# Gaius-Augustus/Augustus

Measured on AMD Instinct MI355X. Metric: Mbp DNA decoded/sec (whole node), ab-initio human model, higher is better.
Workload: dtype f64; 1 GPU; synthetic uniform-random DNA, 100 contigs x 1000000 bp per GPU, --species=human ab initio (47 states, sample=0); pieces_in_flight_per_gpu=100, batches_in_flight_per_gpu=1

## Files before the change

augustus_amd/csrc/device/decoder.hip:

```cpp
#include <hip/hip_runtime.h>
#include <sys/mman.h>
#include <algorithm>
#include <map>
#include <array>
#include <cmath>
#include <unordered_map>
#include <cstdio>
#include <cstdlib>
#include <cstring>
#include <future>
#include <memory>
#include <mutex>
#include <set>
#include <string>
#include <system_error>
#include <thread>
#include <atomic>
#include <chrono>
#include <vector>
#include "kernels.h"
#include "dense.h"
#include "layout.h"
#include "launch.h"
#include "assmemo.h"
// ... 156 lines not shown
    if (t < NF) {
        uint64_t x = L.w[t][0];
        for (int i = 1; i < SCAN_W; i++) x = t < nSum ? x + L.w[t][i] : (x > L.w[t][i] ? x : L.w[t][i]);
        tot[t] = x;
    }
}
template <int NF> __device__ inline void blockScan(uint64_t (&v)[NF], int nSum, ScanLds<NF> &L, const uint64_t *pre) {
    const int t = threadIdx.x, lane = t & 63, wave = t >> 6;
#pragma unroll
    for (int f = 0; f < NF; f++) {
        const uint64_t x = f < nSum ? waveScanIncl<true>(v[f]) : waveScanIncl<false>(v[f]);
        v[f] = x;
        if (lane == 63) L.w[f][wave] = x;
    }
    __syncthreads();
    if (t < NF) {
        uint64_t acc = pre[t];
        for (int i = 0; i < SCAN_W; i++) {
            const uint64_t x = L.w[t][i];
            L.w[t][i] = acc;
            acc = t < nSum ? acc + x : (acc > x ? acc : x);
        }
    }
    __syncthreads();
#pragma unroll
    for (int f = 0; f < NF; f++) {
        const uint64_t a = L.w[f][wave];
        v[f] = f < nSum ? v[f] + a : (v[f] > a ? v[f] : a);
    }
}
constexpr int NSF = NCNT + 6;
__global__ void __launch_bounds__(SCAN_T) kSiteScanTotals(const DevTables *__restrict__ T, BatchView B, uint64_t *tot ) {
    __shared__ ScanLds<NSF> L;
    __shared__ SlotCodes C;
    C.load(B);
    const int64_t g = (int64_t)blockIdx.x * SCAN_T + threadIdx.x;
    uint64_t v[NSF];
    k1SiteTermsCalc(*T, B, g, v, v + NCNT, C.c, C.lo, C.lo + 256 + 2 * SLOT_HALO);
    blockTotals<NSF>(v, NCNT, L, tot + (int64_t)blockIdx.x * NSF);
}
__global__ void __launch_bounds__(SCAN_T) kSiteScanApply(const DevTables *__restrict__ T, BatchView B, const uint64_t *tot) {
    __shared__ ScanLds<NSF> L;
    __shared__ SlotCodes C;
    C.load(B);
    const int64_t g = (int64_t)blockIdx.x * SCAN_T + threadIdx.x;
    uint64_t v[NSF];
    k1SiteTermsCalc(*T, B, g, v, v + NCNT, C.c, C.lo, C.lo + 256 + 2 * SLOT_HALO);
    blockScan<NSF>(v, NCNT, L, tot + (int64_t)blockIdx.x * NSF);
#pragma unroll
    for (int f = 0; f < NCNT; f++) B.cnt[fidx(g, f, NCNT)] = (uint32_t)v[f];
#pragma unroll
    for (int f = 0; f < 6; f++) B.nsm[fidx(g, f, 6)] = (uint32_t)v[NCNT + f];
}
__global__ void __launch_bounds__(SCAN_T) kFxScanTotals(const DevTables *__restrict__ T, BatchView B, uint64_t *tot ) {
    __shared__ ScanLds<NFX> L;
    __shared__ SlotCodes C;
    C.load(B);
    const int64_t g = (int64_t)blockIdx.x * SCAN_T + threadIdx.x;
    uint64_t v[NFX];
    if (!k1FxTermsCalc(*T, B, g, blockIdx.y, v, C.c, C.lo, C.lo + 256 + 2 * SLOT_HALO)) return;
    blockTotals<NFX>(v, NFX, L, tot + ((int64_t)blockIdx.y * (B.N / SCAN_T) + blockIdx.x) * NFX);
}
__global__ void __launch_bounds__(SCAN_T) kFxScanApply(const DevTables *__restrict__ T, BatchView B, const uint64_t *tot) {
    __shared__ ScanLds<NFX> L;
    __shared__ SlotCodes C;
    C.load(B);
    const int64_t g = (int64_t)blockIdx.x * SCAN_T + threadIdx.x;
    uint64_t v[NFX];
    if (!k1FxTermsCalc(*T, B, g, blockIdx.y, v, C.c, C.lo, C.lo + 256 + 2 * SLOT_HALO)) return;
    blockScan<NFX>(v, NFX, L, tot + ((int64_t)blockIdx.y * (B.N / SCAN_T) + blockIdx.x) * NFX);
    uint64_t *fx = B.fx + (int64_t)blockIdx.y * B.N * NFX;
#pragma unroll
    for (int f = 0; f < NFX; f++) fx[fidx(g, f, NFX)] = v[f];
}
__global__ void __launch_bounds__(64) kChunkOffsets(uint64_t *tot, BatchView B, int nf, int nSum) {
    const int p = blockIdx.x, f = blockIdx.z, lane = threadIdx.x;
    tot += (int64_t)blockIdx.y * (B.N / SCAN_T) * nf;
    const bool sum = f < nSum;
    uint64_t acc = 0;
    const int64_t c1 = B.off[p + 1] / SCAN_T;
    for (int64_t c0 = B.off[p] / SCAN_T; c0 < c1; c0 += 64) {
        const int64_t ch = c0 + lane;
        const uint64_t v = ch < c1 ? tot[ch * nf + f] : 0;
        uint64_t x = v;
        for (int o = 1; o < 64; o <<= 1) {
            const uint64_t y = (uint64_t)__shfl_up((unsigned long long)x, o, 64);
            if (lane >= o) x = sum ? x + y : (x > y ? x : y);
        }
        const uint64_t prev = (uint64_t)__shfl_up((unsigned long long)x, 1, 64);
        const uint64_t ex = lane == 0 ? acc : (sum ? acc + prev : (acc > prev ? acc : prev));
        if (ch < c1) tot[ch * nf + f] = ex;
        const uint64_t last = (uint64_t)__shfl((unsigned long long)x, 63, 64);
        acc = sum ? acc + last : (acc > last ? acc : last);
    }
}

constexpr int NUF = NUFX + NUCNT;
__global__ void __launch_bounds__(SCAN_T) kUtrScanTotals(const DevTables *__restrict__ T, BatchView B, uint64_t *tot ) {
    __shared__ ScanLds<NUF> L;
    __shared__ SlotCodes C;
    C.load(B);
    const int64_t g = (int64_t)blockIdx.x * SCAN_T + threadIdx.x;
    uint64_t v[NUF];
    k1UtrTermsCalc(*T, B, g, v, C.c, C.lo, C.lo + 256 + 2 * SLOT_HALO);
    blockTotals<NUF>(v, NUF, L, tot + (int64_t)blockIdx.x * NUF);
}
__global__ void __launch_bounds__(SCAN_T) kUtrScanApply(const DevTables *__restrict__ T, BatchView B, const uint64_t *tot) {
    __shared__ ScanLds<NUF> L;
    __shared__ SlotCodes C;
    C.load(B);
    const int64_t g = (int64_t)blockIdx.x * SCAN_T + threadIdx.x;
    uint64_t v[NUF];
    k1UtrTermsCalc(*T, B, g, v, C.c, C.lo, C.lo + 256 + 2 * SLOT_HALO);
    blockScan<NUF>(v, NUF, L, tot + (int64_t)blockIdx.x * NUF);
#pragma unroll
    for (int f = 0; f < NUFX; f++) B.ufx[fidx(g, f, NUFX)] = v[f];
#pragma unroll
    for (int f = 0; f < NUCNT; f++) B.ucnt[fidx(g, f, NUCNT)] = (uint32_t)v[NUFX + f];
}
__global__ void kUtrListCount(BatchView B) {
    int p = blockIdx.x * blockDim.x + threadIdx.x;
    if (p < B.nPieces) k1UtrListCount(B, p);
// ... 50 lines not shown
    const int t = threadIdx.x;
    if (t == 0) running = 0;
    __syncthreads();
    for (int base = w.b0; base <= w.b1; base += 256) {
        const int q = base + t;
        const uint32_t cnt = q <= w.b1 ? V.blkCnt[(w.gb0 + q) * 2 + 1] : 0;
        sc[t] = cnt;
        __syncthreads();
        for (int off = 1; off < 256; off <<= 1) {
            const uint32_t v = t >= off ? sc[t - off] : 0;
            __syncthreads();
            sc[t] += v;
            __syncthreads();
        }
        const uint64_t dst = (uint64_t)w.poolOff + running + (sc[t] - cnt);
        if (cnt) {
            const Item *src = V.items + V.blkOff[(w.gb0 + q) * 2 + 1];
            for (uint32_t i = 0; i < cnt; i++) outItems[dst + i] = src[i];
        }
        __syncthreads();
        if (t == 255) running += sc[255];
        __syncthreads();
    }
    const int64_t nFx = (int64_t)w.nPl * 2 * w.nSlots;
    for (int64_t i = t; i < nFx; i += 256) {
        const int pl = (int)(i / (2 * w.nSlots)), rev = (int)((i / w.nSlots) % 2), g = w.g0 + (int)(i % w.nSlots);
        outFx[w.fxOff + i] = V.fx[(int64_t)pl * V.N * NFX + fidx(w.o + g, rev ? FX_INR : FX_INF, NFX)];
    }
    if (mat && outF)
        for (int64_t i = t; i < (int64_t)w.nRows * S; i += 256) outF[w.fOff + i] = mat[(w.o + 1 + w.r0) * S + i];
}
__global__ void __launch_bounds__(256) kPatchItems(BatchView B, const uint64_t *idx, const double *te, int n) {
    const int i = blockIdx.x * blockDim.x + threadIdx.x;
    if (i < n) B.items[idx[i]].te = te[i];
}

namespace augx { namespace dev {
#define AUGX_BY_BLK(f, ...) do { if (blk == 8) f##8(__VA_ARGS__); else if (blk == 4) f##4(__VA_ARGS__); else f##2(__VA_ARGS__); } while (0)
void launchTrellis(int blk, int mode, bool ties, unsigned grid, hipStream_t st, const DevTables *T, const BatchView *B) { AUGX_BY_BLK(launchTrellis_, mode, ties, grid, st, T, B); }
void launchCand(int blk, bool multi, bool dense, unsigned grid, hipStream_t st, const DevTables *T, const BatchView &W) { AUGX_BY_BLK(launchCand_, multi, dense, grid, st, T, W); }
void launchForward(int blk, unsigned grid, hipStream_t st, const DevTables *T, const BatchView *B) { AUGX_BY_BLK(launchForward_, grid, st, T, B); }
void launchDense(int blk, int mode, bool ties, unsigned grid, hipStream_t st, const DevTables *T, const BatchView *B) { AUGX_BY_BLK(launchDense_, mode, ties, grid, st, T, B); }
void launchUtrDesc(int blk, unsigned grid, hipStream_t st, const DevTables *T, const BatchView &W) { AUGX_BY_BLK(launchUtrDesc_, grid, st, T, W); }
#undef AUGX_BY_BLK
}}

struct augx_decoder {
    const augx_model *model = nullptr;
    int device = 0;
    hipStream_t stream = nullptr;
    DevTables hostT;
    DevTables *dT = nullptr;
    std::vector<void *> tableBufs;
    bool debugCells = false;
    int blk = 8;
    int nCU = 256;
    int share = 1;
    std::multimap<size_t, void *> pool;
    std::unordered_map<void *, size_t> live;
    std::atomic<size_t> pooledBytes{0};
    std::mutex poolMu;
    std::vector<hipStream_t> copyStreams;
    bool dense = false;
    bool countNearTies = false;
    int64_t nearTies = 0, nearTiePieces = 0;
    double mallocSeconds = 0, mallocBytes = 0;
    bool exactMulti = true;
};

namespace {
int snippetCacheReplay(augx_decoder *d, augx_batch *b, int64_t &nPatched, bool fromLists, const double *mat);
int utrCachesReplay(augx_decoder *d, augx_batch *b, const double *mat, bool &rebuilt);
std::mutex g_regMu;
std::vector<augx_decoder *> g_decoders;
constexpr size_t POOL_CAP_BYTES = (size_t)250 << 30;
size_t sizeClass(size_t bytes) {
    if (bytes < ((size_t)1 << 20)) return (bytes + 4095) & ~(size_t)4095;
    size_t p2 = (size_t)1 << 20;
    while (p2 < bytes) p2 <<= 1;
    const size_t step = p2 >> 4;
    return (bytes + step - 1) / step * step;
}
void poolReleaseLocked(augx_decoder *d) {
    for (auto &kv : d->pool) (void)hipFree(kv.second);
    d->pool.clear();
    d->pooledBytes = 0;
}
void poolRelease(augx_decoder *d) {
    std::lock_guard<std::mutex> lk(d->poolMu);
    poolReleaseLocked(d);
}
hipError_t devMalloc(augx_decoder *d, void **out, size_t bytes) {
    if (bytes == 0) bytes = 1;
    bytes = sizeClass(bytes);
    {
        std::lock_guard<std::mutex> lk(d->poolMu);
        auto it = d->pool.lower_bound(bytes);
        if (it != d->pool.end() && it->first <= bytes + bytes / 4 + 4096) {
            *out = it->second;
            d->live[*out] = it->first;
            d->pooledBytes -= it->first;
            d->pool.erase(it);
            return hipSuccess;
        }
    }
    const auto tm0 = std::chrono::steady_clock::now();
// ... 134 lines not shown

}

extern "C" {

int augx_device_count(void) {
    int ndev = 0;
    if (hipGetDeviceCount(&ndev) != hipSuccess) { (void)hipGetLastError(); return 0; }
    return ndev;
}

int augx_decoder_create(const augx_model *m, int device, augx_decoder **out) {
    if (!m || !out) { setLastError("augx_decoder_create: NULL argument"); return AUGX_E_ARG; }
    *out = nullptr;
    int ndev = 0;
    hipError_t e = hipGetDeviceCount(&ndev);
    if (e != hipSuccess || ndev <= 0) {
        setLastError("augx_decoder_create: no HIP device available (this library has no CPU decode path)");
        return AUGX_E_NODEVICE;
    }
    if (device < 0 || device >= ndev) { setLastError("augx_decoder_create: bad device index"); return AUGX_E_ARG; }
    const augx_tables &t = m->m.t;
    int blk = 8;
    try {
        blk = chooseBlockSize(t);
    } catch (std::exception &ex) {
        setLastError(ex.what());
        return AUGX_E_UNSUPPORTED;
    }
    HIP_TRY(hipSetDevice(device));
    augx_decoder *d = new augx_decoder();
    d->model = m;
    d->device = device;
    d->blk = blk;
    d->dense = modelIsDense(t);
    d->countNearTies = getenv("AUGX_NEAR_TIES") && atoi(getenv("AUGX_NEAR_TIES")) != 0;
    const char *dbg = getenv("AUGX_DEBUG_CELLS");
    d->debugCells = dbg && atoi(dbg) != 0;
    if (const char *ex = getenv("AUGX_EXACT_MULTICLASS")) d->exactMulti = atoi(ex) != 0;
    { int cu = 0; if (hipDeviceGetAttribute(&cu, hipDeviceAttributeMultiprocessorCount, device) == hipSuccess && cu > 0) d->nCU = cu; else (void)hipGetLastError(); }
    const int rc = [&]() -> int {
        HIP_TRY(hipStreamCreate(&d->stream));
        try { fillDevTablesScalars(t, d->hostT); } catch (std::exception &ex) { setLastError(ex.what()); return AUGX_E_UNSUPPORTED; }
        for (auto &sp : tableSpans(t, d->hostT)) {
            void *p = nullptr;
            size_t bytes = (size_t)(sp.count > 0 ? sp.count : 1) * sizeof(double);
            HIP_TRY(hipMalloc(&p, bytes));
            d->tableBufs.push_back(p);
            if (sp.count > 0) HIP_TRY(hipMemcpy(p, sp.src, (size_t)sp.count * sizeof(double), hipMemcpyHostToDevice));
            *sp.dst = (TabPtr)p;
        }
        HIP_TRY(hipMalloc((void **)&d->dT, sizeof(DevTables)));
        HIP_TRY(hipMemcpy(d->dT, &d->hostT, sizeof(DevTables), hipMemcpyHostToDevice));
        return AUGX_OK;
    }();
    if (rc) { augx_decoder_destroy(d); return rc; }
    { std::lock_guard<std::mutex> rk(g_regMu); g_decoders.push_back(d); }
    *out = d;
    return AUGX_OK;
}

int augx_decoder_set_share(augx_decoder *d, int n) {
    if (!d || n < 1) { setLastError("augx_decoder_set_share: bad argument"); return AUGX_E_ARG; }
    d->share = n;
    return AUGX_OK;
}

int augx_decoder_count_near_ties(augx_decoder *d, int on) { if (!d) return AUGX_E_ARG; d->countNearTies = on != 0; return AUGX_OK; }
int64_t augx_decoder_near_ties(const augx_decoder *d, int64_t *pieces) { if (pieces) *pieces = d ? d->nearTiePieces : 0; return d ? d->nearTies : 0; }
int augx_decoder_exact(const augx_decoder *d) { return d && d->exactMulti ? 1 : 0; }
int augx_decoder_set_exact(augx_decoder *d, int on) {
    if (!d) return AUGX_E_ARG;
    d->exactMulti = on != 0;
    return AUGX_OK;
}

int64_t augx_decoder_batch_capacity(augx_decoder *d) {
    if (!d) return 0;
    size_t freeB = 0, totalB = 0;
    if (hipSetDevice(d->device) != hipSuccess || hipMemGetInfo(&freeB, &totalB) != hipSuccess) return 16L * 1000 * 1000;
    freeB += d->pooledBytes;
    {
        size_t nOn = 0;
        std::lock_guard<std::mutex> rk(g_regMu);
        for (augx_decoder *o : g_decoders) nOn += o->device == d->device;
        if (nOn > 1) freeB = std::min(freeB, (size_t)((double)totalB * 0.9 / (double)nOn));
    }
    int64_t cap = (int64_t)(freeB / (d->dense ? 1500 + 18 * (size_t)d->model->m.t.S : d->model->m.t.n_classes > 1 ? 2000 : 1500));
    if (cap > 128L * 1000 * 1000) cap = 128L * 1000 * 1000;
    if (cap < 1000 * 1000) cap = 1000 * 1000;
    return cap;
}

int64_t augx_decoder_sampled_capacity(augx_decoder *d) {
    const int64_t cap = augx_decoder_batch_capacity(d);
    if (!d || d->dense) return cap;
    const int64_t base = d->model->m.t.n_classes > 1 ? 2000 : 1500;
    return cap * base / (base + 8 * (int64_t)d->model->m.t.S);
}

void augx_release_host_pools();
void augx_decoder_destroy(augx_decoder *d) {
    if (!d) return;
    bool last;
    { std::lock_guard<std::mutex> rk(g_regMu); g_decoders.erase(std::remove(g_decoders.begin(), g_decoders.end(), d), g_decoders.end()); last = g_decoders.empty(); }
    if (last) augx_release_host_pools();
// ... 218 lines not shown
            HIP_TRY(hipMemcpy(planeCls.data(), V.planeCls, sizeof(int32_t) * n * MAXPL, hipMemcpyDeviceToHost));
            std::vector<uint8_t> wc, plane;
            for (int p = 0; p < n; p++) {
                if (cls[p] >= 0) continue;
                const int len = b->L.len[p];
                wc.resize((size_t)len);
                HIP_TRY(hipMemcpy(wc.data(), V.gcRaw + b->L.off[p] + 1, (size_t)len, hipMemcpyDeviceToHost));
                const int np = stairsPlanes(wc.data(), len, d->model->m.t.gc_win, plane, &planeCls[(size_t)p * MAXPL]);
                if (np < 0) continue;
                cls[p] = planeCls[(size_t)p * MAXPL];
                nPlanes[p] = np;
                if (np > nPl) nPl = np;
                if (np > 1) HIP_TRY(hipMemcpy(V.gcPlane + b->L.off[p] + 1, plane.data(), (size_t)len, hipMemcpyHostToDevice));
            }
            HIP_TRY(hipMemcpy(V.cls, cls.data(), sizeof(int32_t) * n, hipMemcpyHostToDevice));
            HIP_TRY(hipMemcpy(V.nPlanes, nPlanes.data(), sizeof(int32_t) * n, hipMemcpyHostToDevice));
            HIP_TRY(hipMemcpy(V.planeCls, planeCls.data(), sizeof(int32_t) * n * MAXPL, hipMemcpyHostToDevice));
        }
        bool changed = W.nPl != nPl;
        if (d->dense && !b->listsReady) {
            utrScan();
            hipLaunchKernelGGL(kUtrListCount, dim3((n + 63) / 64), dim3(64), 0, st, V);
            HIP_TRY(hipGetLastError());
            HIP_TRY(hipStreamSynchronize(st));
        }
        if (!b->listsReady) {
            std::vector<int32_t> lc(n);
            std::vector<int64_t> offs;
            HIP_TRY(hipMemcpy(lc.data(), V.listCnt, sizeof(int32_t) * n, hipMemcpyDeviceToHost));
            W.listCap = listOffsets(lc.data(), n, offs);
            b->hListOffs = offs;
            HIP_TRY(hipMemcpy(b->dListOffs, offs.data(), sizeof(int64_t) * (n + 1), hipMemcpyHostToDevice));
            b->listsReady = true;
            changed = true;
        }
        bool grown = false;
        if (timingFirst) tf[2] = nowS();
        if ((rc = ensureArrays(b, nPl, W.listCap, &grown))) return rc;
        if (timingFirst) tf[3] = nowS();
        if (changed || grown) {
            W.nPl = nPl;
            HIP_TRY(hipMemcpy(b->dV, &W, sizeof(BatchView), hipMemcpyHostToDevice));
        }
    }
    }
    if (V.nPl > b->chunkTotPlanes) {
        DevBuf nt;
        if ((rc = nt.alloc(d, sizeof(uint64_t) * (size_t)V.nPl * (V.N / SCAN_T) * NFX, "augx_batch_decode: out of device memory for the scan totals"))) return rc;
        b->V.chunkTot = nt.as<uint64_t>();
        b->bufs.push_back(std::move(nt));
        b->chunkTotPlanes = V.nPl;
    }
    if (d->dense && !b->utrScanned) utrScan();
    hipLaunchKernelGGL(kFxScanTotals, dim3(nScan, V.nPl), dim3(SCAN_T), 0, st, d->dT, V, V.chunkTot);
    hipLaunchKernelGGL(kChunkOffsets, dim3(n, V.nPl, NFX), dim3(64), 0, st, V.chunkTot, V, NFX, NFX);
    hipLaunchKernelGGL(kFxScanApply, dim3(nScan, V.nPl), dim3(SCAN_T), 0, st, d->dT, V, V.chunkTot);
    hipLaunchKernelGGL(kSignals, dim3(gridN), dim3(256), 0, st, d->dT, V);
    hipLaunchKernelGGL(kSiteSignals, dim3((unsigned)((V.listCap + 255) / 256), 4), dim3(256), 0, st, d->dT, V);
    hipLaunchKernelGGL(kSiteConsts, dim3(gridN, V.nPl), dim3(256), 0, st, d->dT, V);
    if (d->dense) hipLaunchKernelGGL(kUtrSignals, dim3(gridN), dim3(256), 0, st, d->dT, V);
    HIP_TRY(hipGetLastError());
    {
        BatchView &W = b->V;
        const unsigned nWg = (unsigned)(W.N / (WAVE * NWAVES));
        if (b->itemBuf && b->nItems > 0 && (uint64_t)W.itemCap > b->nItems + b->nItems / 16 + 65536) {
            HIP_TRY(hipStreamSynchronize(st));
            b->itemBuf.reset();
            b->itemsVerified = false;
        }
        if (!b->itemBuf) {
            W.itemCap = b->nItems > 0 ? (int64_t)(b->nItems + b->nItems / 16 + 65536) : W.N * 18 + 65536;
            if ((rc = b->itemBuf.alloc(d, (size_t)W.itemCap * sizeof(Item), "augx_batch_decode: out of device memory for the candidate buffer; decode fewer bases per batch"))) return rc;
            W.items = b->itemBuf.as<Item>();
            HIP_TRY(hipMemcpyAsync(b->dV, &W, sizeof(BatchView), hipMemcpyHostToDevice, st));
        }
        const bool utrDesc = d->dense && d->hostT.utr;
        if (utrDesc && !b->udBuf) {
            W.udCap = b->nDescs > 0 ? (int64_t)(b->nDescs + 64) : W.N / 2 + 65536;
            if (const char *e = getenv("AUGX_UD_CAP")) { if (b->nDescs == 0) W.udCap = atol(e) > 0 ? atol(e) : 1; }
            if ((rc = b->udBuf.alloc(d, (size_t)W.udCap * sizeof(UDesc), "augx_batch_decode: out of device memory for the UTR descriptors; decode fewer bases per batch"))) return rc;
            W.ud = b->udBuf.as<UDesc>();
            HIP_TRY(hipMemcpyAsync(b->dV, &W, sizeof(BatchView), hipMemcpyHostToDevice, st));
        }
        const bool steady = b->decoded && b->itemBuf && b->nItems > 0 && (uint64_t)W.itemCap >= b->nItems && b->itemsVerified;
        for (int attempt = 0;; attempt++) {
            HIP_TRY(hipMemsetAsync(W.candAlloc, 0, sizeof(CandAlloc), st));
            const bool multi = W.nPl > 1;
            if (utrDesc) {
                const unsigned nGrp = (unsigned)(W.N / (NT / 16));
                launchUtrDesc(d->blk, nGrp, st, d->dT, W);
            }
            launchCand(d->blk, multi, d->dense, nWg, st, d->dT, W);
            HIP_TRY(hipGetLastError());
            if (steady) break;
            CandAlloc tot;
            HIP_TRY(hipMemcpyAsync(&tot, W.candAlloc, sizeof tot, hipMemcpyDeviceToHost, st));
            HIP_TRY(hipStreamSynchronize(st));
            b->nPairs = tot.pairs; b->nItems = tot.items; b->nDescs = tot.descs;
            const bool itemsFit = (int64_t)tot.items <= W.itemCap, descsFit = !utrDesc || (int64_t)tot.descs <= W.udCap;
            if (itemsFit && descsFit) { b->itemsVerified = true; break; }
            if (attempt > 0) { setLastError("augx_batch_decode: candidate buffers overflowed twice"); return AUGX_E_HIP; }
            if (!itemsFit) {
                W.itemCap = (int64_t)tot.items + 64;
                if ((rc = b->itemBuf.alloc(d, (size_t)W.itemCap * sizeof(Item), "augx_batch_decode: out of device memory for the candidate buffer (" + std::to_string(tot.items) + " candidates); decode fewer bases per batch"))) return rc;
                W.items = b->itemBuf.as<Item>();
            }
            if (!descsFit) {
                W.udCap = (int64_t)tot.descs + 64;
                if ((rc = b->udBuf.alloc(d, (size_t)W.udCap * sizeof(UDesc), "augx_batch_decode: out of device memory for the UTR descriptors; decode fewer bases per batch"))) return rc;
// ... 1017 lines not shown
```

augustus_amd/csrc/device/kernels.h:

```cpp
#pragma once
#include <type_traits>
#include "dp.h"

namespace augx {
namespace dev {

#ifdef AUGX_EMU
#define FOR_LANES(l) for (int l = 0; l < WAVE; ++l)
#define LV(T, name) T name[WAVE]
#define LV2(T, name, K) T name[K][WAVE]
#define LI l
#define LX(name) name[l]
#define WAVE_SYNC() ((void)0)
#define GLOBAL_SYNC() ((void)0)
#define AUGX_KFN inline
#define FOR_THREADS(t) for (int t = 0; t < NT; ++t)
#define FOR_WAVES(w) for (int w = 0; w < NWAVES; ++w)
#define FOR_WLANES(t, w) for (int t = (w) * WAVE; t < (w) * WAVE + WAVE; ++t)
#define TV(T, name) T name[NT]
#define TV2(T, name, K) T name[K][NT]
#define TI t
#define TX(name) name[t]
#define BLOCK_SYNC() ((void)0)
#define BLOCK_GLOBAL_SYNC() ((void)0)
// ... 185 lines not shown
}
AUGX_HD int k1WindowClass(const DevTables &T, const BatchView &B, int64_t g) {
    int p = B.chunkPiece[g / CHUNK];
    int64_t o = B.off[p];
    int s = (int)(g - o - 1), n = B.len[p];
    int win = T.gc_win;
    if (win > n || win < 1) win = n;
    if (s < 0 || s > n - win) return -1;
    if (T.C == 1) { B.gcRaw[g] = 0; return 0; }
    double cnt[4];
    for (int i = 0; i < 4; i++) cnt[i] = (double)(B.cnt[fidx(o + s + win, i, NCNT)] - B.cnt[fidx(o + s, i, NCNT)]);
    if (cnt[0] + cnt[1] + cnt[2] + cnt[3] == 0.0)
        for (int i = 0; i < 4; i++) cnt[i] = (double)(B.cnt[fidx(o + win, i, NCNT)] - B.cnt[fidx(o, i, NCNT)]);
    const int c = nearestClass(T, cnt);
    B.gcRaw[g] = (uint8_t)c;
    return c;
}

AUGX_HD bool k1FxTermsCalc(const DevTables &T, const BatchView &B, int64_t g, int pl, uint64_t out[NFX],
                           const uint8_t *lcode = nullptr, int lLo = 0, int lHi = 0) {
    int p = B.chunkPiece[g / CHUNK];
    if (pl > 0 && pl >= B.nPlanes[p]) return false;
    int64_t o = B.off[p];
    int q = (int)(g - o - 1);
    for (int i = 0; i < NFX; i++) out[i] = 0;
    Piece P;
    P.t = &T; P.n = B.len[p]; P.c = B.cls[p] < 0 ? -1 : B.planeCls[p * MAXPL + pl]; P.o = o; P.code = B.code + o + 1; P.fx = nullptr; P.nsm = nullptr; P.sig = nullptr;
    P.lcode = lcode; P.lLo = lLo; P.lHi = lHi;
    if (q >= 0 && q < B.len[p] && P.c >= 0) {
    const int k = T.k, NP = T.NP, c = P.c;
    int pn = q >= k ? P.pat(q - k, k + 1) : -1;
    int rn = P.rcpat(q, k + 1);
    const double *tabs[3] = {T.ex_emi + (int64_t)c * 3 * NP, T.ex_init + (int64_t)c * 3 * NP, T.ex_et + (int64_t)c * 3 * NP};
    for (int a = 0; a < 3; a++)
        for (int tb = 0; tb < 3; tb++) {
            out[(0 * 3 + a) * 3 + tb] = toFx(pn >= 0 ? tabs[tb][mod3(q + a) * NP + pn] : T.ln_n_coding);
            out[(1 * 3 + a) * 3 + tb] = toFx(rn >= 0 ? tabs[tb][mod3(a - q) * NP + rn] : T.ln_n_coding);
        }
    const double *inE = T.in_emi + (int64_t)c * T.NPin;
    const double softB = (T.soft && B.raw[g] >= 'a' && B.raw[g] <= 'z') ? T.lnSoft : 0.0;
    const int ki = T.kIn;
    const int pni = ki == k ? pn : (q >= ki ? P.pat(q - ki, ki + 1) : -1);
    out[FX_INF] = toFx((pni >= 0 ? inE[pni] : T.ln_quarter) + softB);
    int rn2 = (q + ki < P.n) ? (ki == k ? rn : P.rcpat(q, ki + 1)) : -1;
    out[FX_INR] = toFx((rn2 >= 0 ? inE[rn2] : T.ln_quarter) + softB);
    }
    return true;
}
AUGX_HD void k1FxTerms(const DevTables &T, const BatchView &B, int64_t g, int pl) {
    uint64_t out[NFX];
    if (!k1FxTermsCalc(T, B, g, pl, out)) return;
    uint64_t *fx = B.fx + (int64_t)pl * B.N * NFX;
    for (int i = 0; i < NFX; i++) fx[fidx(g, i, NFX)] = out[i];
}

constexpr int NSITE = 4;
AUGX_HD void k1Signals(const DevTables &T, const BatchView &B, int64_t g, const uint8_t *lcode = nullptr, int lLo = 0, int lHi = 0) {
    int p = B.chunkPiece[g / CHUNK];
    int64_t o = B.off[p];
    int q = (int)(g - o - 1);
    double e[NSIG];
    for (int i = 0; i < NSIG; i++) e[i] = AUGX_NINF;
    int32_t stv[NSITE];
    for (int i = 0; i < NSITE; i++) stv[i] = -1;
    uint64_t gate = 0;
    int64_t atgIdx = -1;
    const bool inPiece = !(q < 0 || q >= B.len[p] || B.cls[p] < 0);
    int64_t lo = 0;
    if (inPiece) {
    Piece P = makePieceAt(T, B, p, B.gcPlane[g]);
    P.lcode = lcode; P.lLo = lLo; P.lHi = lHi;
    const double softB = (T.soft && B.raw[g] >= 'a' && B.raw[g] <= 'z') ? T.lnSoft : 0.0;
    e[SIG_EIG] = q >= 1 ? eIg(P, q) + softB : AUGX_NINF;
    e[SIG_EIN] = eIn(P, q) + softB;
    if (T.utr && T.uk != T.k) e[SIG_EUIN] = eUin(P, q) + softB;
    e[SIG_TISR] = tisRev(P, q);
    e[SIG_STOPF] = exEndPart(P, AUGX_K_TERMINAL, 0, q, AUGX_NINF);
    uint64_t cn[NCNT], cp[NCNT];
    for (int i = CNT_ATG; i < NCNT; i++) { cn[i] = B.cnt[fidx(g, i, NCNT)]; cp[i] = B.cnt[fidx(g - 1, i, NCNT)]; }
    lo = listOff(B, p);
    for (int i = 0; i < NSITE; i++)
        stv[i] = cn[CNT_LA + i] != cp[CNT_LA + i] ? (int32_t)cn[CNT_LA + i] - 1 : -1;
    if (cn[CNT_ATG] != cp[CNT_ATG]) atgIdx = (int64_t)cn[CNT_ATG] - 1;
    if (q - T.dStateLen >= 0) e[SIG_EQD] = P.seg(FX_INF, q - T.dStateLen + 1, q);
    if (q >= 1) {
        const bool stopOpen = e[SIG_STOPF] > AUGX_NINF && q - 3 >= 0;
        const bool tisOpen = e[SIG_TISR] > AUGX_NINF && q - T.W - 3 >= 0;
        bool fwdOpen[3];
        for (int w2 = 0; w2 < 3; w2++) fwdOpen[w2] = exEndPart(P, AUGX_K_INTERNAL, w2, q, AUGX_NINF) > AUGX_NINF;
        const bool revOpen = exEndPart(P, AUGX_K_RINTERNAL, 0, q, AUGX_NINF) > AUGX_NINF;
        const bool lessOpen = lessDGate(P, true, q), rlessOpen = lessDGate(P, false, q);
        for (int s = 0; s < T.S; s++) {
            if (!T.reachable[s]) continue;
            const int kind = T.kind[s], w2 = T.win[s];
            bool open = false;
            switch (kind) {
            case AUGX_K_SINGLE: case AUGX_K_TERMINAL: open = stopOpen; break;
            case AUGX_K_RSINGLE: case AUGX_K_RINITIAL: open = tisOpen; break;
            case AUGX_K_INITIAL: case AUGX_K_INTERNAL: open = w2 == 0 ? fwdOpen[0] : w2 == 1 ? fwdOpen[1] : fwdOpen[2]; break;
            case AUGX_K_RINTERNAL: case AUGX_K_RTERMINAL: open = revOpen; break;
            case AUGX_K_LESSD: open = lessOpen; break;
            case AUGX_K_RLESSD: open = rlessOpen; break;
            default: break;
            }
            if (open) gate |= 1ull << T.vbit[s];
        }
// ... 2565 lines not shown
        }
    }
}

AUGX_KFN void segFinalizePiece(const BatchView &B, int p) {
    const int s0 = B.pieceSeg0[p], K = B.pieceSeg0[p + 1] - s0, n = B.len[p];
    if (K <= 1) {
        B.brkPos[s0] = n - 1; B.brkOff[s0] = 0.0;
        if (B.status[p] == 0 && !(fabs(B.lnv[p]) < AUGX_EXACT_LIMIT)) B.status[p] = AUGX_E_RANGE;
        return;
    }
    double off = 0.0;
    int covered = -1, r = 0;
    bool abortAny = false;
    const int lastTile = (n + WAVE - 1) / WAVE - 1;
    for (int k = 0; k < K; k++)
        if (B.segStatus[s0 + k]) abortAny = true;
    for (int k = 1; k < K; k++) {
        const int st = B.segStop[s0 + k];
        int endTile = st >= -1 ? st : B.segStop2[s0 + k];
        const double D = st >= -1 ? B.segD[s0 + k] : B.segD2[s0 + k];
        if (st < -1 && endTile < 0) { abortAny = true; endTile = lastTile; }
#ifdef AUGX_EMU
        if (endTile < covered - 1) g_emuTrellis[ET_FIN_OVERRUN]++;
        else { g_emuTrellis[ET_FIN_COVERED] += st < -1 && endTile > covered; g_emuTrellis[endTile >= lastTile ? ET_FIN_TO_END : ET_FIN_SEAM]++; }
#endif
        if (endTile < covered - 1) continue;
        if (st < -1 && endTile > covered) covered = endTile;
        if (endTile >= lastTile) break;
        B.brkPos[s0 + r] = (endTile + 1) * WAVE - 1; B.brkOff[s0 + r] = off; r++;
        off = off + D;
    }
    for (; r < K; r++) { B.brkPos[s0 + r] = n - 1; B.brkOff[s0 + r] = off; }
    if (B.status[p] == 0) B.lnv[p] = B.lnv[p] + off;
    if (abortAny) B.status[p] = AUGX_E_HIP;
    if (B.status[p] == 0 && !(fabs(B.lnv[p]) < AUGX_EXACT_LIMIT)) B.status[p] = AUGX_E_RANGE;
}

#ifdef AUGX_EMU
inline int waveCount(const int *flag) { int c = 0; for (int l = 0; l < WAVE; l++) c += flag[l] != 0; return c; }
inline int waveFirstTrue(const int *flag) {
    for (int l = 0; l < WAVE; l++)
        if (flag[l]) return l;
    return WAVE;
}
#else
__device__ inline int waveCount(const int *flag) { return __popcll(__ballot(flag[0] != 0)); }
__device__ inline int waveFirstTrue(const int *flag) {
    unsigned long long m = __ballot(flag[0] != 0);
    return m ? (int)__ffsll((long long)m) - 1 : WAVE;
}
#endif

AUGX_KFN void backtracePiece(const DevTables &T, const BatchView &B, int p) {
    const int n = B.len[p];
    const int64_t o = B.off[p];
    const int64_t po = pathOff(B, p), cap = pathCap(B, p);
    int state = B.finalState[p];
    int base = n - 1;
    int count = 0, nearTies = 0;
    bool overflow = false;
    if (state < 0 || B.status[p] != 0) {
        FOR_LANES(l) { if (l == 0) { B.pathCount[p] = 0; if (B.nearTie) B.nearTie[p] = 0; } }
        return;
    }
    const int dssWhole = T.Ds + 2 + T.De, assLag = T.As + 2 + T.Ae + T.U;
    const bool segmented = B.pieceSeg0[p + 1] - B.pieceSeg0[p] > 1;
    while (base > 0) {
        const int kind = T.kind[state];
        int eop, ai;
        const bool chain = kind == AUGX_K_IGENIC || kind == AUGX_K_GEOMETRIC || kind == AUGX_K_RGEOMETRIC;
        if (chain) {
            int selfAi = -1;
            for (int i = 0; i < T.n_anc[state]; i++)
                if (T.anc[state][i] == state) selfAi = i;
            int cur = base;
            uint16_t w = BP_NONE;
            int cslot = 0;
            for (int s2 = 0; s2 < state; s2++)
                if (T.reachable[s2] && (T.kind[s2] == AUGX_K_IGENIC || T.kind[s2] == AUGX_K_GEOMETRIC || T.kind[s2] == AUGX_K_RGEOMETRIC)) cslot++;
            for (;;) {
                LV(int, flag);
                LV(int, wv);
                LV(int, hit);
                FOR_LANES(l) {
                    LX(flag) = 0; LX(wv) = -1; LX(hit) = 4;
#pragma unroll
                    for (int k = 3; k >= 0; k--) {
                        const int q = cur - 4 * l - k;
                        const int raw = q >= 1 ? (int)B.bpChain[(o + 1 + q) * 8 + cslot] : -1;
                        const int ww = raw < 0 || raw == 0xFF ? raw : (raw & 0x7F);
                        if (q < 1 || ww != selfAi) { LX(flag) = 1; LX(wv) = ww; LX(hit) = k; }
                    }
                }
                int first = waveFirstTrue(flag);
                if (first < WAVE) {
#ifdef AUGX_EMU
                    const int hk = hit[first], hw = wv[first];
#else
                    const int hk = __shfl(hit[0], first, 64), hw = __shfl(wv[0], first, 64);
#endif
                    cur -= 4 * first + hk;
                    w = cur >= 1 ? (uint16_t)hw : BP_NONE;
                    break;
                }
                cur -= 4 * WAVE;
            }
            if (B.nearTie) {
                const int lo2 = cur < 1 ? 1 : cur;
                for (int q0 = lo2; q0 <= base; q0 += WAVE) {
                    LV(int, fl);
                    FOR_LANES(l) { const int q = q0 + l; LX(fl) = (q <= base && B.bpChain[(o + 1 + q) * 8 + cslot] != 0xFF && (B.bpChain[(o + 1 + q) * 8 + cslot] & 0x80)) ? 1 : 0; }
                    nearTies += waveCount(fl);
                }
            }
            if (cur < 1) { eop = 0; ai = -1; }
            else { eop = cur - 1; ai = w; }
        } else if ((kind >= AUGX_K_SINGLE && kind <= AUGX_K_RTERMINAL) || kind == AUGX_K_LESSD || kind == AUGX_K_RLESSD) {
            const int blkSz = B.blk;
            const int64_t gb = o / blkSz + base / blkSz;
            const uint64_t i0 = B.blkOff[gb * 2 + 1];
            const uint32_t cnt = B.blkCnt[gb * 2 + 1], pid = (uint32_t)(((base % blkSz) << 6) | state);
            Best best{AUGX_NINF, -2147483647, -1};
            double runnerUp = AUGX_NINF;
            for (int pass = 0; pass < (B.nearTie ? 2 : 1); pass++)
            for (uint32_t c0 = 0; c0 < cnt; c0 += WAVE) {
                LV(double, cv);
                LV(int, ck);
                LV(int, ca);
                FOR_LANES(l) {
                    LX(cv) = AUGX_NINF; LX(ck) = -2147483647; LX(ca) = -1;
                    const uint32_t it = c0 + (uint32_t)l;
                    if (it < cnt) {
                        const Item I = B.items[i0 + it];
                        if ((I.kp >> KEY_BITS) == pid && I.te > AUGX_NINF) {
                            const uint32_t sr = I.src, tag = sr >> 30;
                            const int sel = (sr >> 26) & 3, fr = (sr >> 24) & 3, pay = (int)(sr & 0xFFFFFFu);
                            double pv;
                            if (tag == SRC_LIST) {
                                const double *a = sel == 0 ? B.laVal : sel == 1 ? B.lrVal : sel == 2 ? B.ldVal : B.rdVal;
                                pv = a[(listOff(B, p) + pay) * 3 + fr];
                                if (segmented) {
                                    const int64_t e = listOff(B, p) + pay;
                                    const int pos = sel == 0 ? B.laPos[e] : sel == 1 ? B.lrPos[e] : sel == 2 ? B.ldEnt[e].pos : B.rdEnt[e].pos;
                                    pv = pv + frameOff(B, p, pos);
                                }
                            } else if (tag == SRC_VIG) {
                                pv = B.vig[o + 1 + pay];
                                if (segmented) pv = pv + frameOff(B, p, pay);
                            } else {
                                const int a0 = (int)(sr & 0x3Fu);
                                pv = B.initKind[p] == 0 ? T.ln_init[a0] : (a0 == T.synch ? 0.0 : AUGX_NINF);
                            }
                            LX(cv) = pv + I.te; LX(ck) = (int)(I.kp & KEY_MASK); LX(ca) = (int)((sr >> 28) & 3);
                            if (pass == 1 && LX(ck) == best.key && LX(ca) == best.aux) LX(cv) = AUGX_NINF;
                        }
                    }
                }
                const Best b2 = waveArgMax(cv, ck, ca);
                if (pass == 0) { if (better(b2.v, b2.key, best.v, best.key)) best = b2; }
                else if (b2.v > runnerUp) runnerUp = b2.v;
            }
            if (B.nearTie && runnerUp > AUGX_NINF && best.v - runnerUp < AUGX_NEAR_TIE && best.v != runnerUp) nearTies++;
            if (!(best.v > AUGX_NINF)) { overflow = true; break; }
            ai = best.aux;
            eop = best.key - KEY_BIAS;
#ifdef AUGX_EMU
// ... 37 lines not shown
```

Baseline: 513.4 Mbp/s.

## Precompute fixed-point emission tables and widen backtrace chain scan rounds

Adds a one-time kernel that converts the exon/intron emission log-probabilities to fixed-point records laid out per pattern. The fx scan kernels then read nine contiguous entries per pattern instead of indexing several double tables and converting each value. Separately, the chain backtrace now loads 64-bit words holding all eight chain slots, covers 2048 positions per round, and folds the near-tie count into the same pass. This adds per-decoder table memory and keeps more values in registers per lane during backtrace.

```diff
diff --git a/augustus_amd/csrc/device/decoder.hip b/augustus_amd/csrc/device/decoder.hip
--- a/augustus_amd/csrc/device/decoder.hip
+++ b/augustus_amd/csrc/device/decoder.hip
@@ -232,22 +232,26 @@
 #pragma unroll
     for (int f = 0; f < 6; f++) B.nsm[fidx(g, f, 6)] = (uint32_t)v[NCNT + f];
 }
-__global__ void __launch_bounds__(SCAN_T) kFxScanTotals(const DevTables *__restrict__ T, BatchView B, uint64_t *tot ) {
+__global__ void __launch_bounds__(256) kFxTabs(const DevTables *__restrict__ T, uint64_t *out, int64_t n) {
+    const int64_t i = (int64_t)blockIdx.x * 256 + threadIdx.x;
+    if (i < n) out[i] = fxTabEntry(*T, i);
+}
+__global__ void __launch_bounds__(SCAN_T) kFxScanTotals(const DevTables *__restrict__ T, FxTabs X, BatchView B, uint64_t *tot ) {
     __shared__ ScanLds<NFX> L;
     __shared__ SlotCodes C;
     C.load(B);
     const int64_t g = (int64_t)blockIdx.x * SCAN_T + threadIdx.x;
     uint64_t v[NFX];
-    if (!k1FxTermsCalc(*T, B, g, blockIdx.y, v, C.c, C.lo, C.lo + 256 + 2 * SLOT_HALO)) return;
+    if (!k1FxTermsRec(*T, X, B, g, blockIdx.y, v, C.c, C.lo, C.lo + 256 + 2 * SLOT_HALO)) return;
     blockTotals<NFX>(v, NFX, L, tot + ((int64_t)blockIdx.y * (B.N / SCAN_T) + blockIdx.x) * NFX);
 }
-__global__ void __launch_bounds__(SCAN_T) kFxScanApply(const DevTables *__restrict__ T, BatchView B, const uint64_t *tot) {
+__global__ void __launch_bounds__(SCAN_T) kFxScanApply(const DevTables *__restrict__ T, FxTabs X, BatchView B, const uint64_t *tot) {
     __shared__ ScanLds<NFX> L;
     __shared__ SlotCodes C;
     C.load(B);
     const int64_t g = (int64_t)blockIdx.x * SCAN_T + threadIdx.x;
     uint64_t v[NFX];
-    if (!k1FxTermsCalc(*T, B, g, blockIdx.y, v, C.c, C.lo, C.lo + 256 + 2 * SLOT_HALO)) return;
+    if (!k1FxTermsRec(*T, X, B, g, blockIdx.y, v, C.c, C.lo, C.lo + 256 + 2 * SLOT_HALO)) return;
     blockScan<NFX>(v, NFX, L, tot + ((int64_t)blockIdx.y * (B.N / SCAN_T) + blockIdx.x) * NFX);
     uint64_t *fx = B.fx + (int64_t)blockIdx.y * B.N * NFX;
 #pragma unroll
@@ -404,6 +408,7 @@
     DevTables hostT;
     DevTables *dT = nullptr;
     std::vector<void *> tableBufs;
+    FxTabs fxTabs{};
     bool debugCells = false;
     int blk = 8;
     int nCU = 256;
@@ -644,6 +649,18 @@
         }
         HIP_TRY(hipMalloc((void **)&d->dT, sizeof(DevTables)));
         HIP_TRY(hipMemcpy(d->dT, &d->hostT, sizeof(DevTables), hipMemcpyHostToDevice));
+        {
+            const int64_t nEx = (int64_t)d->hostT.C * d->hostT.NP * FXREC, nIn = (int64_t)d->hostT.C * d->hostT.NPin, nAll = nEx + 2 * nIn + 3;
+            uint64_t *p = nullptr, tail[3];
+            HIP_TRY(hipMalloc((void **)&p, (size_t)nAll * sizeof(uint64_t)));
+            d->tableBufs.push_back(p);
+            hipLaunchKernelGGL(kFxTabs, dim3((unsigned)((nAll + 255) / 256)), dim3(256), 0, d->stream, d->dT, p, nAll);
+            HIP_TRY(hipGetLastError());
+            HIP_TRY(hipMemcpyAsync(tail, p + nEx + 2 * nIn, sizeof(tail), hipMemcpyDeviceToHost, d->stream));
+            HIP_TRY(hipStreamSynchronize(d->stream));
+            d->fxTabs.ex = p; d->fxTabs.in = p + nEx;
+            d->fxTabs.nCoding = tail[0]; d->fxTabs.quarter[0] = tail[1]; d->fxTabs.quarter[1] = tail[2];
+        }
         return AUGX_OK;
     }();
     if (rc) { augx_decoder_destroy(d); return rc; }
@@ -968,9 +985,9 @@
         b->chunkTotPlanes = V.nPl;
     }
     if (d->dense && !b->utrScanned) utrScan();
-    hipLaunchKernelGGL(kFxScanTotals, dim3(nScan, V.nPl), dim3(SCAN_T), 0, st, d->dT, V, V.chunkTot);
+    hipLaunchKernelGGL(kFxScanTotals, dim3(nScan, V.nPl), dim3(SCAN_T), 0, st, d->dT, d->fxTabs, V, V.chunkTot);
     hipLaunchKernelGGL(kChunkOffsets, dim3(n, V.nPl, NFX), dim3(64), 0, st, V.chunkTot, V, NFX, NFX);
-    hipLaunchKernelGGL(kFxScanApply, dim3(nScan, V.nPl), dim3(SCAN_T), 0, st, d->dT, V, V.chunkTot);
+    hipLaunchKernelGGL(kFxScanApply, dim3(nScan, V.nPl), dim3(SCAN_T), 0, st, d->dT, d->fxTabs, V, V.chunkTot);
     hipLaunchKernelGGL(kSignals, dim3(gridN), dim3(256), 0, st, d->dT, V);
     hipLaunchKernelGGL(kSiteSignals, dim3((unsigned)((V.listCap + 255) / 256), 4), dim3(256), 0, st, d->dT, V);
     hipLaunchKernelGGL(kSiteConsts, dim3(gridN, V.nPl), dim3(256), 0, st, d->dT, V);
diff --git a/augustus_amd/csrc/device/kernels.h b/augustus_amd/csrc/device/kernels.h
--- a/augustus_amd/csrc/device/kernels.h
+++ b/augustus_amd/csrc/device/kernels.h
@@ -261,6 +261,65 @@
     if (!k1FxTermsCalc(T, B, g, pl, out)) return;
     uint64_t *fx = B.fx + (int64_t)pl * B.N * NFX;
     for (int i = 0; i < NFX; i++) fx[fidx(g, i, NFX)] = out[i];
+}
+
+constexpr int FXREC = 9;
+struct FxTabs {
+    const uint64_t *ex;
+    const uint64_t *in;
+    uint64_t nCoding;
+    uint64_t quarter[2];
+};
+AUGX_HD uint64_t fxTabEntry(const DevTables &T, int64_t i) {
+    const int64_t nEx = (int64_t)T.C * T.NP * FXREC, nIn = (int64_t)T.C * T.NPin;
+    if (i < nEx) {
+        const int64_t cp = i / FXREC;
+        const int tb = (int)(i % FXREC) / 3, fr = (int)(i % FXREC) % 3, c = (int)(cp / T.NP), pn = (int)(cp % T.NP);
+        const TabPtr tab = tb == 0 ? T.ex_emi : tb == 1 ? T.ex_init : T.ex_et;
+        return toFx(tab[((int64_t)c * 3 + fr) * T.NP + pn]);
+    }
+    i -= nEx;
+    if (i < 2 * nIn) return toFx(T.in_emi[i % nIn] + (i < nIn ? 0.0 : T.lnSoft));
+    i -= 2 * nIn;
+    return i == 0 ? toFx(T.ln_n_coding) : toFx(T.ln_quarter + (i == 1 ? 0.0 : T.lnSoft));
+}
+AUGX_HD bool k1FxTermsRec(const DevTables &T, const FxTabs &X, const BatchView &B, int64_t g, int pl, uint64_t out[NFX],
+                          const uint8_t *lcode = nullptr, int lLo = 0, int lHi = 0) {
+    int p = B.chunkPiece[g / CHUNK];
+    if (pl > 0 && pl >= B.nPlanes[p]) return false;
+    int64_t o = B.off[p];
+    int q = (int)(g - o - 1);
+    for (int i = 0; i < NFX; i++) out[i] = 0;
+    Piece P;
+    P.t = &T; P.n = B.len[p]; P.c = B.cls[p] < 0 ? -1 : B.planeCls[p * MAXPL + pl]; P.o = o; P.code = B.code + o + 1; P.fx = nullptr; P.nsm = nullptr; P.sig = nullptr;
+    P.lcode = lcode; P.lLo = lLo; P.lHi = lHi;
+    if (q >= 0 && q < B.len[p] && P.c >= 0) {
+    const int k = T.k, c = P.c;
+    const int pn = q >= k ? P.pat(q - k, k + 1) : -1;
+    const int rn = P.rcpat(q, k + 1);
+    const int r = mod3(q);
+    uint64_t f[FXREC], v[FXREC];
+    const uint64_t *fr = X.ex + ((int64_t)c * T.NP + (pn >= 0 ? pn : 0)) * FXREC, *rr = X.ex + ((int64_t)c * T.NP + (rn >= 0 ? rn : 0)) * FXREC;
+    for (int i = 0; i < FXREC; i++) { f[i] = fr[i]; v[i] = rr[i]; }
+    for (int tb = 0; tb < 3; tb++) {
+        const uint64_t f0 = pn >= 0 ? f[tb * 3] : X.nCoding, f1 = pn >= 0 ? f[tb * 3 + 1] : X.nCoding, f2 = pn >= 0 ? f[tb * 3 + 2] : X.nCoding;
+        const uint64_t v0 = rn >= 0 ? v[tb * 3] : X.nCoding, v1 = rn >= 0 ? v[tb * 3 + 1] : X.nCoding, v2 = rn >= 0 ? v[tb * 3 + 2] : X.nCoding;
+        out[(0 * 3 + 0) * 3 + tb] = r == 0 ? f0 : r == 1 ? f1 : f2;
+        out[(0 * 3 + 1) * 3 + tb] = r == 0 ? f1 : r == 1 ? f2 : f0;
+        out[(0 * 3 + 2) * 3 + tb] = r == 0 ? f2 : r == 1 ? f0 : f1;
+        out[(1 * 3 + 0) * 3 + tb] = r == 0 ? v0 : r == 1 ? v2 : v1;
+        out[(1 * 3 + 1) * 3 + tb] = r == 0 ? v1 : r == 1 ? v0 : v2;
+        out[(1 * 3 + 2) * 3 + tb] = r == 0 ? v2 : r == 1 ? v1 : v0;
+    }
+    const int soft = (T.soft && B.raw[g] >= 'a' && B.raw[g] <= 'z') ? 1 : 0;
+    const uint64_t *inE = X.in + ((int64_t)soft * T.C + c) * T.NPin;
+    const int ki = T.kIn;
+    const int pni = ki == k ? pn : (q >= ki ? P.pat(q - ki, ki + 1) : -1);
+    out[FX_INF] = pni >= 0 ? inE[pni] : X.quarter[soft];
+    const int rn2 = (q + ki < P.n) ? (ki == k ? rn : P.rcpat(q, ki + 1)) : -1;
+    out[FX_INR] = rn2 >= 0 ? inE[rn2] : X.quarter[soft];
+    }
+    return true;
 }
 
 constexpr int NSITE = 4;
@@ -2932,6 +2991,7 @@
 }
 #endif
 
+constexpr int BT_ROUND = 2048;
 AUGX_KFN void backtracePiece(const DevTables &T, const BatchView &B, int p) {
     const int n = B.len[p];
     const int64_t o = B.off[p];
@@ -2959,40 +3019,50 @@
             int cslot = 0;
             for (int s2 = 0; s2 < state; s2++)
                 if (T.reachable[s2] && (T.kind[s2] == AUGX_K_IGENIC || T.kind[s2] == AUGX_K_GEOMETRIC || T.kind[s2] == AUGX_K_RGEOMETRIC)) cslot++;
+            const auto chain8 = gp((const uint64_t *)B.bpChain) + o + 1;
             for (;;) {
-                LV(int, flag);
+                LV2(uint64_t, cb, BT_ROUND / WAVE);
+                LV(int, hd);
                 LV(int, wv);
-                LV(int, hit);
                 FOR_LANES(l) {
-                    LX(flag) = 0; LX(wv) = -1; LX(hit) = 4;
-#pragma unroll
-                    for (int k = 3; k >= 0; k--) {
-                        const int q = cur - 4 * l - k;
-                        const int raw = q >= 1 ? (int)B.bpChain[(o + 1 + q) * 8 + cslot] : -1;
-                        const int ww = raw < 0 || raw == 0xFF ? raw : (raw & 0x7F);
-                        if (q < 1 || ww != selfAi) { LX(flag) = 1; LX(wv) = ww; LX(hit) = k; }
+#pragma unroll
+                    for (int j = 0; j < BT_ROUND / WAVE / 2; j++) {
+                        const int q1 = cur - 2 * WAVE * j - 2 * l - 1;
+                        const auto at = chain8 + (q1 < 0 ? 0 : q1);
+                        cb[2 * j + 1][LI] = at[0]; cb[2 * j][LI] = at[1];
                     }
                 }
-                int first = waveFirstTrue(flag);
-                if (first < WAVE) {
-#ifdef AUGX_EMU
-                    const int hk = hit[first], hw = wv[first];
-#else
-                    const int hk = __shfl(hit[0], first, 64), hw = __shfl(wv[0], first, 64);
-#endif
-                    cur -= 4 * first + hk;
+                FOR_LANES(l) {
+                    LX(hd) = BT_ROUND; LX(wv) = -1;
+#pragma unroll
+                    for (int i = BT_ROUND / WAVE - 1; i >= 0; i--) {
+                        const int d = WAVE * (i & ~1) + 2 * l + (i & 1), q = cur - d;
+                        const int raw = (int)(cb[i][LI] >> (8 * cslot)) & 0xFF;
+                        const int ww = raw == 0xFF ? raw : (raw & 0x7F);
+                        if (q < 1 || ww != selfAi) { LX(hd) = d; LX(wv) = q < 1 ? -1 : ww; }
+                    }
+                }
+                const int dmin = waveMin(hd, 0);
+                if (B.nearTie) {
+                    LV(int, nt);
+                    FOR_LANES(l) {
+                        LX(nt) = 0;
+#pragma unroll
+                        for (int i = 0; i < BT_ROUND / WAVE; i++) {
+                            const int d = WAVE * (i & ~1) + 2 * l + (i & 1), raw = (int)(cb[i][LI] >> (8 * cslot)) & 0xFF;
+                            LX(nt) += (d <= dmin && cur - d >= 1 && raw != 0xFF && (raw & 0x80)) ? 1 : 0;
+                        }
+                    }
+                    waveInclScan(nt, 0);
+                    nearTies += waveRead(nt, 0, WAVE - 1);
+                }
+                if (dmin < BT_ROUND) {
+                    const int hw = waveRead(wv, 0, (dmin % (2 * WAVE)) >> 1);
+                    cur -= dmin;
                     w = cur >= 1 ? (uint16_t)hw : BP_NONE;
                     break;
                 }
-                cur -= 4 * WAVE;
-            }
-            if (B.nearTie) {
-                const int lo2 = cur < 1 ? 1 : cur;
-                for (int q0 = lo2; q0 <= base; q0 += WAVE) {
-                    LV(int, fl);
-                    FOR_LANES(l) { const int q = q0 + l; LX(fl) = (q <= base && B.bpChain[(o + 1 + q) * 8 + cslot] != 0xFF && (B.bpChain[(o + 1 + q) * 8 + cslot] & 0x80)) ? 1 : 0; }
-                    nearTies += waveCount(fl);
-                }
+                cur -= BT_ROUND;
             }
             if (cur < 1) { eop = 0; ai = -1; }
             else { eop = cur - 1; ai = w; }
```

Result: faster. 528.7 Mbp/s (median of 6 runs) (+3.0%).
